# ViTAE-Transformer/SAMRS

Hardware: AMD Instinct MI355X
Metric: images/sec (1024^2, vit_h, 32 boxes/img) SAM box->mask (higher is better)
Workload: dtype f16

## Files before the change

samrs_amd/csrc/engine.hip:

```cpp
#include <algorithm>
#include <cmath>
#include <cstdarg>
#include <cstdio>
#include <cstring>
#include <map>
#include <mutex>
#include <utility>
#include <cstdlib>
#include <string>
#include <vector>

#include "../../include/samrs_hip.h"
#include "../../include/samrs_hip_internal.h"
#include "common.h"
#include "kernels.h"

namespace {

struct DevTensor {
    float* p = nullptr;
    std::vector<int64_t> shape;
    size_t numel = 0;
};

// ... 122 lines not shown

    std::vector<DecLayer> layers;
    DecAttn fin{};
    DecWeights dec{};
    uint16_t* fin_kv_w = nullptr;
    float *fin_kv_b = nullptr, *fin_pe = nullptr;
    uint16_t *up1_w = nullptr, *up2_w = nullptr, *up1_w_lo = nullptr, *up2_w_lo = nullptr;
    float *up1_b = nullptr, *up2_b = nullptr, *up_ln = nullptr;
    float* PE = nullptr;

    float *TOK0 = nullptr, *Q = nullptr, *TA = nullptr, *TQ = nullptr, *TK = nullptr, *TV = nullptr, *TO = nullptr;
    float *MH = nullptr, *QP = nullptr, *KT = nullptr, *VT = nullptr, *O128 = nullptr, *T2IW = nullptr;
    float *K0F = nullptr;
    uint16_t* K0E = nullptr;
    uint16_t* KVQ0 = nullptr;
    float* KF = nullptr;
    uint16_t* KE = nullptr;
    uint16_t* KE_lo = nullptr;
    float* DENSE = nullptr;
    int* SLOT_OF = nullptr;
    uint16_t* KVQ = nullptr;
    uint16_t* OI = nullptr;
    float* U1raw = nullptr;
    uint16_t* U1 = nullptr;
    uint16_t* U2 = nullptr;
    float *HY1 = nullptr, *HY2 = nullptr, *HYPER = nullptr, *IOU = nullptr, *LOW = nullptr;

    void* rle_scratch = nullptr;
    size_t rle_scratch_bytes = 0;
    void* region_scratch = nullptr;
// ... 303 lines not shown
    {
        DeviceGuard dg(device);
        if (dg.status != hipSuccess) return bad("hipSetDevice failed (no HIP device? this library has no CPU fallback)");
    }
    samrs_engine* e = new samrs_engine();
    e->cfg = *cfg;
    e->device = device;
    e->prec = cfg->precision;
    e->grid = cfg->img_size / cfg->patch_size;
    e->tokens = e->grid * e->grid;
    e->D = cfg->embed_dim;
    e->C = cfg->out_chans;
    e->hd = hd;
    e->nwin = (e->grid + cfg->window_size - 1) / cfg->window_size;
    e->T_max = 5 + cfg->max_points + 1 + 2;
    e->slot_set.assign(cfg->max_images, 0);
    e->slot_split.assign(cfg->max_images, 0);
    e->slot_depth.assign(cfg->max_images, 0);
    e->decoder_fusion = env_int("SAMRS_DECODER_FUSION", 1) != 0;
    e->ln_fold = env_int("SAMRS_LN_FOLD", 0) != 0 && gemm_has_experiments();
    const bool h_like = gemm_split3_ok(e->tokens, 3 * e->D, e->D) && gemm_split3_ok(e->tokens, e->D, e->D) && (2 * e->D) % 320 == 0;
    e->split = env_int("SAMRS_SPLIT", SPLIT_DEFAULT | (h_like ? SPLIT_ATTN_V : 0)) & SPLIT_ALL;
    e->grade_multimask = h_like ? SPLIT_ATTN_ANY : 0;
    e->allow_reduced = env_int("SAMRS_ALLOW_REDUCED", getenv("SAMRS_SPLIT") ? 1 : 0) != 0;
    e->upscaler_fused = env_int("SAMRS_UPSCALER_FUSED", 1) != 0;
    e->split_passes = env_int("SAMRS_SPLIT_PASSES", 0) != 0;
    e->split_depth = env_int("SAMRS_SPLIT_DEPTH", 0);
    e->lo_format = (h_like && env_int("SAMRS_LO_FORMAT", 4) == 4) ? 4 : 0;
    e->gelu_fast = env_int("SAMRS_GELU_FAST", -1);
    e->ln_tail = env_int("SAMRS_LN_TAIL", 0) != 0;
// ... 53 lines not shown
        tmp.resize(t.numel);
        for (int64_t ci = 0; ci < Ci; ++ci)
            for (int64_t co = 0; co < Co; ++co)
                for (int64_t s = 0; s < 4; ++s) tmp[(s * Co + co) * Ci + ci] = host[(ci * Co + co) * 4 + s];
        src = tmp.data();
    }
    auto it = e->w.find(n);
    if (it != e->w.end()) return fail(e, SAMRS_ERR_BAD_WEIGHTS, "duplicate tensor %s", name);
    CK(e, dalloc(e, &t.p, t.numel));
    CK(e, hipMemcpy(t.p, src, t.numel * sizeof(float), hipMemcpyHostToDevice));
    e->w.emplace(n, std::move(t));
    return SAMRS_OK;
}

static void audit_build_sites(samrs_engine_t* e);

int samrs_finalize_weights(samrs_engine_t* e, void* stream) {
    if (!e) return SAMRS_ERR_BAD_ARG;
    if (e->finalized) return SAMRS_OK;
    hipStream_t s = (hipStream_t)stream;
    ON_DEVICE(e);
    std::vector<std::pair<std::string, std::vector<int64_t>>> req;
    required_tensors(e, req);
    for (auto& r : req) {
        auto it = e->w.find(r.first);
        if (it == e->w.end()) return fail(e, SAMRS_ERR_BAD_WEIGHTS, "missing tensor %s", r.first.c_str());
        if (it->second.shape != r.second) return fail(e, SAMRS_ERR_BAD_WEIGHTS, "shape mismatch for %s", r.first.c_str());
    }
    if (e->w.size() != req.size()) {
        for (auto& kv : e->w) {
// ... 152 lines not shown
    CK(e, dalloc(e, &e->fin_pe, (size_t)tokens * 2 * Ci));
    CK(e, hipMemsetAsync(e->fin_pe, 0, sizeof(float) * tokens * 2 * Ci, s));
    CK(e, launch_gemm_f32(e->PE, C, e->fin.kw, nullptr, e->fin_pe, 2 * Ci, tokens, Ci, C, false, false, s));
    if ((rc = to_et(e, "mask_decoder.output_upscaling.0.weight", &e->up1_w, false, s, &e->up1_w_lo))) return rc;
    if ((rc = to_et(e, "mask_decoder.output_upscaling.3.weight", &e->up2_w, false, s, &e->up2_w_lo))) return rc;
    CK(e, dalloc(e, &e->up1_b, (size_t)C));
    CK(e, dalloc(e, &e->up2_b, (size_t)C / 2));
    CK(e, dalloc(e, &e->up_ln, (size_t)C / 2));
    CK(e, hipMemcpyAsync(e->up_ln, W(e, "mask_decoder.output_upscaling.1.weight"), sizeof(float) * C / 4, hipMemcpyDeviceToDevice, s));
    CK(e, hipMemcpyAsync(e->up_ln + C / 4, W(e, "mask_decoder.output_upscaling.1.bias"), sizeof(float) * C / 4, hipMemcpyDeviceToDevice, s));
    for (int k = 0; k < 4; ++k) {
        CK(e, hipMemcpyAsync(e->up1_b + k * (C / 4), W(e, "mask_decoder.output_upscaling.0.bias"), sizeof(float) * C / 4, hipMemcpyDeviceToDevice, s));
        CK(e, hipMemcpyAsync(e->up2_b + k * (C / 8), W(e, "mask_decoder.output_upscaling.3.bias"), sizeof(float) * C / 8, hipMemcpyDeviceToDevice, s));
    }

    const size_t Bi = c.max_images, Bb = c.max_prompts;
    const size_t M = Bi * tokens;
    const size_t Mmax = M;
    CK(e, dalloc(e, &e->X, M * D));
    CK(e, dalloc(e, &e->ln_counters, M / 256 + 1));
    CK(e, hipMemsetAsync(e->ln_counters, 0, (M / 256 + 1) * sizeof(unsigned int), s));
    const size_t y_ld_max = e->ldk ? (size_t)e->ldk : (e->outlier_blocks ? (size_t)D + 64 : (size_t)D);
    CK(e, dalloc(e, &e->Y, Mmax * y_ld_max));
    CK(e, hipMemsetAsync(e->Y, 0, Mmax * y_ld_max * 2, s));
    if (e->can_fold) { CK(e, dalloc(e, &e->STATS, Mmax * 16)); CK(e, dalloc(e, &e->ROWSTAT, Mmax * 2)); }
    CK(e, dalloc(e, &e->QKV, Mmax * 3 * D));
    CK(e, dalloc(e, &e->AO, M * D));
    CK(e, dalloc(e, &e->VTG, M * D));
    if (e->oc_resid) {
        CK(e, dalloc(e, &e->OCX, M * 64));
        if (!(e->split & SPLIT_ATTN_ANY)) CK(e, dalloc(e, &e->AOlo, M * D));
// ... 15 lines not shown
                if (!e->Y4[h]) {
                CK(e, dalloc(e, &e->Y4[h], M * D / 2)); CK(e, dalloc(e, &e->SY4[h], mx_scale_bytes((int)M, D, false)));
                }
                CK(e, dalloc(e, &e->AO4[h], M * e->mx_kp_proj / 2)); CK(e, dalloc(e, &e->SAO4[h], mx_scale_bytes((int)M, e->mx_kp_proj, false)));
            }
        }
        if (e->split & SPLIT_MLP) CK(e, dalloc(e, &e->Hlo, M * 4 * D));
    }
    size_t hsz = M * 4 * D;
    if (M * 9 * C * 2 > hsz) hsz = M * 9 * C * 2;
    if (M * 768 > hsz) hsz = M * 768;
    CK(e, dalloc(e, &e->H, hsz));
    CK(e, dalloc(e, &e->N1, M * C));
    CK(e, dalloc(e, &e->N1e, M * C));
    CK(e, dalloc(e, &e->EMB, M * C));
    const size_t BT = Bb * e->T_max;
    CK(e, dalloc(e, &e->TOK0, BT * C)); CK(e, dalloc(e, &e->Q, BT * C)); CK(e, dalloc(e, &e->TA, BT * C));
    CK(e, dalloc(e, &e->TQ, BT * C)); CK(e, dalloc(e, &e->TK, BT * C)); CK(e, dalloc(e, &e->TV, BT * C));
    CK(e, dalloc(e, &e->TO, BT * C)); CK(e, dalloc(e, &e->MH, BT * 2048));
    CK(e, dalloc(e, &e->QP, BT * Ci)); CK(e, dalloc(e, &e->KT, BT * Ci)); CK(e, dalloc(e, &e->VT, BT * Ci));
    CK(e, dalloc(e, &e->O128, BT * Ci));
    CK(e, dalloc(e, &e->T2IW, t2i_workspace_floats(c.max_prompts, e->T_max)));
    CK(e, dalloc(e, &e->K0F, (size_t)c.max_images * tokens * C)); CK(e, dalloc(e, &e->K0E, (size_t)c.max_images * tokens * C));
    CK(e, dalloc(e, &e->KVQ0, (size_t)c.max_images * tokens * 3 * (C / 2)));
    CK(e, dalloc(e, &e->KF, Bb * tokens * C)); CK(e, dalloc(e, &e->KE, Bb * tokens * C));
    CK(e, dalloc(e, &e->KE_lo, Bb * tokens * C));
    CK(e, dalloc(e, &e->KVQ, Bb * tokens * 3 * Ci)); CK(e, dalloc(e, &e->OI, Bb * tokens * Ci));
    CK(e, dalloc(e, &e->U1raw, Bb * tokens * C)); CK(e, dalloc(e, &e->U1, Bb * tokens * C));
    CK(e, dalloc(e, &e->U2, Bb * tokens * 4 * (C / 2)));
    CK(e, dalloc(e, &e->HY1, 5 * Bb * C)); CK(e, dalloc(e, &e->HY2, 5 * Bb * C));
    CK(e, dalloc(e, &e->HYPER, Bb * 4 * (C / 8))); CK(e, dalloc(e, &e->IOU, Bb * 4));
    CK(e, dalloc(e, &e->LOW, Bb * 3 * 256 * 256));
    CK(e, hipStreamSynchronize(s));
    e->dec = dec_weights(e);
    audit_build_sites(e);
    e->finalized = true;
    return SAMRS_OK;
}

static int prepare_slot_keys(samrs_engine_t* e, int slot0, int n, hipStream_t s);

enum { AUDIT_QKV_IN = 0, AUDIT_Q, AUDIT_K, AUDIT_V, AUDIT_PROJ_IN, AUDIT_LIN1_IN, AUDIT_LIN2_IN, AUDIT_PER_BLOCK };
enum { AUDIT_NECK1_IN = 0, AUDIT_NECK2_IN, AUDIT_KEYS0, AUDIT_TAIL };

static void audit_build_sites(samrs_engine_t* e) {
    static const char* const per_block[AUDIT_PER_BLOCK] = {"qkv_in", "q", "k", "v", "proj_in", "lin1_in", "lin2_in"};
    e->audit_sites.clear();
// ... 564 lines not shown
                         : fail(e, SAMRS_ERR_CAPACITY, "slot out of range");
        if (!e->slot_set[slot])
            return multi ? fail(e, SAMRS_ERR_NOT_SET, "An image must be set with .set_image(...) before mask prediction "
                                "(image %d: slot %d is not set).", i, slot)
                         : fail(e, SAMRS_ERR_NOT_SET, "An image must be set with .set_image(...) before mask prediction.");
    }
    if (!boxes && !point_coords && !mask_input) return fail(e, SAMRS_ERR_BAD_ARG, "at least one prompt (points, boxes or mask_input) is required");
    if (point_coords && !point_labels) return fail(e, SAMRS_ERR_BAD_ARG, "point_labels must be supplied if point_coords is supplied.");
    if (point_coords && (n_points < 1 || n_points > c.max_points)) return fail(e, SAMRS_ERR_CAPACITY, "n_points=%d exceeds max_points=%d", n_points, c.max_points);
    for (int i = 0; i < n_img; ++i)
        if (im[i].in_h < 1 || im[i].in_w < 1 || im[i].in_h > c.img_size || im[i].in_w > c.img_size || im[i].orig_h < 1 || im[i].orig_w < 1)
            return multi ? fail(e, SAMRS_ERR_BAD_SHAPE, "image %d: bad input/original size", i) : fail(e, SAMRS_ERR_BAD_SHAPE, "bad input/original size");
    return SAMRS_OK;
}

static int predict_images(samrs_engine_t* e, const PredictImage* im, int n_img, const float* boxes, const float* point_coords,
                          const int32_t* point_labels, int n_points, const float* mask_input, int multimask, int return_logits,
                          float* iou_out, float* lowres_out, void* stream) {
    const int cap = e->cfg.max_prompts;
    const size_t nsel = multimask ? 3 : 1;
    const int np = point_coords ? n_points : 0;
    const int n = n_img ? im[n_img - 1].p1 : 0;
    std::vector<PredictImage> seg;
    int first = 0;
    for (int off = 0; off < n; off += cap) {
        const int m = (n - off) < cap ? (n - off) : cap;
        seg.clear();
        for (int i = first; i < n_img && im[i].p0 < off + m; ++i) {
            const int a = im[i].p0 > off ? im[i].p0 : off, b = im[i].p1 < off + m ? im[i].p1 : off + m;
            if (b <= a) continue;
            PredictImage sgm = im[i];
            const size_t mask_stride = nsel * (size_t)im[i].orig_h * (size_t)im[i].orig_w * (return_logits ? 4 : 1);
            sgm.p0 = a - off; sgm.p1 = b - off;
            sgm.masks = im[i].masks ? (void*)((unsigned char*)im[i].masks + (size_t)(a - im[i].p0) * mask_stride) : nullptr;
// ... 7 lines not shown
            iou_out ? iou_out + (size_t)off * nsel : nullptr, lowres_out ? lowres_out + (size_t)off * nsel * 256 * 256 : nullptr, stream);
        if (rc) return rc;
    }
    return SAMRS_OK;
}

int samrs_predict(samrs_engine_t* e, int slot, int n, const float* boxes, const float* point_coords,
                  const int32_t* point_labels, int n_points, const float* mask_input, int multimask,
                  int return_logits, int in_h, int in_w, int orig_h, int orig_w, void* masks_out, float* iou_out,
                  float* lowres_out, void* stream) {
    if (!e) return SAMRS_ERR_BAD_ARG;
    if (n < 1) return fail(e, SAMRS_ERR_BAD_ARG, "n_prompts must be >= 1");
    if (multimask) { const int rc = check_multimask_grade(e, slot, false); if (rc != SAMRS_OK) return rc; }
    const PredictImage im{slot, 0, n, in_h, in_w, orig_h, orig_w, masks_out};
    { const int rc = check_predict(e, &im, 1, false, boxes, point_coords, point_labels, n_points, mask_input); if (rc != SAMRS_OK) return rc; }
    return predict_images(e, &im, 1, boxes, point_coords, point_labels, n_points, mask_input, multimask, return_logits, iou_out,
                          lowres_out, stream);
}

int samrs_predict_multi(samrs_engine_t* e, int n_images, const int* slots, const int* prompt_offsets, const float* boxes,
                        const float* point_coords, const int32_t* point_labels, int n_points, const float* mask_input, int multimask,
                        int return_logits, const int* in_hw, const int* orig_hw, void* const* masks_out, float* iou_out,
                        float* lowres_out, void* stream) {
    if (!e) return SAMRS_ERR_BAD_ARG;
    if (n_images < 1 || !slots || !prompt_offsets || !in_hw || !orig_hw)
        return fail(e, SAMRS_ERR_BAD_ARG, "samrs_predict_multi: n_images must be >= 1 and slots, prompt_offsets, in_hw, orig_hw non-null");
    if (prompt_offsets[0] != 0) return fail(e, SAMRS_ERR_BAD_ARG, "samrs_predict_multi: prompt_offsets[0] must be 0, got %d", prompt_offsets[0]);
    std::vector<PredictImage> im((size_t)n_images);
    for (int i = 0; i < n_images; ++i) {
        if (prompt_offsets[i + 1] < prompt_offsets[i])
            return fail(e, SAMRS_ERR_BAD_ARG, "samrs_predict_multi: prompt_offsets must not decrease (image %d: %d -> %d)", i,
                        prompt_offsets[i], prompt_offsets[i + 1]);
        im[i] = PredictImage{slots[i], prompt_offsets[i], prompt_offsets[i + 1], in_hw[2 * i], in_hw[2 * i + 1], orig_hw[2 * i],
                             orig_hw[2 * i + 1], masks_out ? masks_out[i] : nullptr};
    }
    if (multimask)
        for (int i = 0; i < n_images; ++i) { const int rc = check_multimask_grade(e, slots[i], true); if (rc != SAMRS_OK) return rc; }
    { const int rc = check_predict(e, im.data(), n_images, true, boxes, point_coords, point_labels, n_points, mask_input); if (rc != SAMRS_OK) return rc; }
    return predict_images(e, im.data(), n_images, boxes, point_coords, point_labels, n_points, mask_input, multimask, return_logits,
                          iou_out, lowres_out, stream);
}

namespace {

enum class I2T { FUSED, PER_SEGMENT, SHARED_RESIDUAL, ACCUMULATE };
enum class Upscaler { ONE_KERNEL, GLN_SPLIT, GLN, UNFUSED };

struct DecodeLayerRoute {
    bool shared = false;
    long bstride = 0;
    bool tab = false;
    I2T i2t = I2T::FUSED;
    bool write_kf = false;
    bool write_ke_lo = false;
// ... 55 lines not shown

static hipError_t ln_tokens(samrs_engine_t* e, int BT, const float* gw, const float* gb, hipStream_t s) {
    return launch_layernorm(e->prec, e->Q, gw, gb, 1e-5f, nullptr, e->Q, BT, e->C, 0, e->grid, 0, s);
}

}

static int run_prompt_side(samrs_engine_t* e, const DecodeRoute& r, const PredictImage* seg, int n_seg, int n, const float* boxes,
                           const float* point_coords, const int32_t* point_labels, int n_points, const float* mask_input, hipStream_t s) {
    const samrs_config& c = e->cfg;
    const int C = e->C, tokens = e->tokens;
    PromptParams pp = e->dec.prompt;
    prompt_call_fields(pp, boxes, point_coords, point_labels, n, n_points, (float)c.img_size);
    CK(e, launch_prompt_tokens(pp, e->TOK0, e->Q, r.T, s));
    if (r.slot_table) {
        if (!e->SLOT_OF) CK(e, dalloc(e, &e->SLOT_OF, (size_t)c.max_prompts));
        std::vector<int> start((size_t)n_seg + 1), slot((size_t)n_seg);
        for (int k = 0; k < n_seg; ++k) { start[k] = seg[k].p0; slot[k] = seg[k].slot; }
        start[n_seg] = seg[n_seg - 1].p1;
        CK(e, launch_fill_slot_table(start.data(), slot.data(), n_seg, e->SLOT_OF, s));
    }
    if (!r.shared0) {
        if (!e->DENSE) CK(e, dalloc(e, &e->DENSE, (size_t)c.max_prompts * tokens * C));
        CK(e, launch_mask_embed(e->dec.mask_embed, mask_input, e->DENSE, n, e->grid, s));
        CK(e, launch_make_keys(e->prec, e->EMB + r.slot0 * tokens * C, e->DENSE, nullptr, e->KF, e->KE, n, tokens, C, s,
                               r.slot_table ? e->SLOT_OF : nullptr));
    }
    return SAMRS_OK;
}

static int run_dec_layer(samrs_engine_t* e, const DecodeRoute& r, int li, const PredictImage* seg, int n_seg, int n, hipStream_t s) {
    const int C = e->C, Ci = C / 2, tokens = e->tokens, prec = e->prec, g = e->grid, T = r.T, BT = r.BT, Mi = r.Mi;
    const DecLayer& L = e->layers[li];
    const DecodeLayerRoute& l = r.layer[li];
    const float* k0f = e->K0F + r.slot0 * tokens * C;
    const uint16_t* kvq = l.shared ? e->KVQ0 + r.slot0 * tokens * 3 * Ci : e->KVQ;
    const int* tab = l.tab ? e->SLOT_OF : nullptr;
    {
// ... 50 lines not shown
}

static int run_final_attn(samrs_engine_t* e, const DecodeRoute& r, int n, hipStream_t s) {
    const int C = e->C, Ci = C / 2, tokens = e->tokens, BT = r.BT;
    CK(e, gemm_f32_sum(e->Q, e->TOK0, C, e->fin.qw, e->fin.qb, e->QP, Ci, BT, Ci, C, s));
    CK(e, launch_gemm_et(e->prec, e->KE, e->fin_kv_w, e->KVQ, e->fin_kv_b, e->fin_pe, tokens, r.Mi, 2 * Ci, C, false, false, false, s));
    CK(e, launch_t2i_attention(e->prec, e->QP, e->KVQ, e->KVQ + Ci, 2 * Ci, tokens, e->O128, e->T2IW, n, r.T, tokens, Ci, 8, s));
    CK(e, launch_gemm_f32(e->O128, Ci, e->fin.ow, e->fin.ob, e->Q, C, BT, C, Ci, false, true, s));
    CK(e, ln_tokens(e, BT, e->dec.norm_final_w, e->dec.norm_final_b, s));
    return SAMRS_OK;
}

static int run_heads(samrs_engine_t* e, const DecodeRoute& r, int n, float* iou_out, hipStream_t s) {
    const int C = e->C;
    const DecWeights& w = e->dec;
    const size_t hs = (size_t)e->cfg.max_prompts * C;
    F32Batch l0{}, l1{}, l2{};
    for (int i = 0; i < 5; ++i) {
        l0.A[i] = i < 4 ? e->Q + (size_t)(1 + i) * C : e->Q;
        l0.W[i] = w.head_w[i][0]; l0.bias[i] = w.head_b[i][0]; l0.C[i] = e->HY1 + i * hs;
        l1.A[i] = e->HY1 + i * hs;
        l1.W[i] = w.head_w[i][1]; l1.bias[i] = w.head_b[i][1]; l1.C[i] = e->HY2 + i * hs;
        if (i < 4) {
            l2.A[i] = e->HY2 + i * hs;
            l2.W[i] = w.head_w[i][2]; l2.bias[i] = w.head_b[i][2]; l2.C[i] = e->HYPER + i * (C / 8);
        }
    }
    CK(e, launch_gemm_f32_batch(l0, 5, r.T * C, C, n, C, C, true, false, s));
    CK(e, launch_gemm_f32_batch(l1, 5, C, C, n, C, C, true, false, s));
    CK(e, launch_gemm_f32_batch(l2, 4, C, 4 * (C / 8), n, C / 8, C, false, false, s));
    if (r.iou)
        CK(e, launch_gemm_f32(e->HY2 + 4 * hs, C, w.head_w[4][2] + (size_t)r.sel0 * C, w.head_b[4][2] + r.sel0, iou_out, r.nsel, n, r.nsel, C,
                              false, false, s));
    return SAMRS_OK;
}

static int run_upscaler(samrs_engine_t* e, const DecodeRoute& r, int n, float* low, hipStream_t s) {
    const int C = e->C, prec = e->prec, g = e->grid, Mi = r.Mi;
    switch (r.up) {
    case Upscaler::ONE_KERNEL:
        CK(e, launch_upscaler_fused(prec, e->KE, r.sp_up ? e->KE_lo : nullptr, e->up1_w, r.sp_up ? e->up1_w_lo : nullptr, e->up1_b, e->up_ln,
                                    e->up2_w, r.sp_up ? e->up2_w_lo : nullptr, e->up2_b, e->HYPER, low, n, g, 4, r.sel0, r.nsel, s));
        break;
    case Upscaler::GLN_SPLIT:
        CK(e, launch_gemm_et_gln(prec, e->KE, e->up1_w, e->U1raw, e->up1_b, e->up_ln, Mi, C, C, s, e->KE_lo, e->up1_w_lo));
        CK(e, launch_upscale2_masks(prec, e->U1raw, e->up2_w, e->up2_w_lo, e->up2_b, e->HYPER, low, n, g, 4, r.sel0, r.nsel, s));
        break;
    case Upscaler::GLN:
        CK(e, launch_gemm_et_gln(prec, e->KE, e->up1_w, e->U1, e->up1_b, e->up_ln, Mi, C, C, s));
        CK(e, launch_upscale2_masks(prec, e->U1, e->up2_w, nullptr, e->up2_b, e->HYPER, low, n, g, 4, r.sel0, r.nsel, s));
        break;
    case Upscaler::UNFUSED:
        CK(e, launch_gemm_et(prec, e->KE, e->up1_w, e->U1raw, e->up1_b, nullptr, 0, Mi, C, C, true, false, false, s));
// ... 5 lines not shown
    return SAMRS_OK;
}

static int run_postprocess(samrs_engine_t* e, const DecodeRoute& r, const PredictImage* seg, int n_seg, const float* low, int return_logits,
                           hipStream_t s) {
    for (int k = 0; k < n_seg; ++k)
        if (seg[k].masks)
            CK(e, launch_postprocess(low + (size_t)seg[k].p0 * r.nsel * 256 * 256, (seg[k].p1 - seg[k].p0) * r.nsel, seg[k].in_h, seg[k].in_w,
                                     seg[k].orig_h, seg[k].orig_w, e->cfg.img_size, return_logits, seg[k].masks, s));
    return SAMRS_OK;
}

static int predict_chunk(samrs_engine_t* e, const PredictImage* seg, int n_seg, int n, const float* boxes, const float* point_coords,
                         const int32_t* point_labels, int n_points, const float* mask_input, int multimask,
                         int return_logits, float* iou_out, float* lowres_out, void* stream) {
    const samrs_config& c = e->cfg;
    if (n < 1 || n > c.max_prompts) return fail(e, SAMRS_ERR_CAPACITY, "n_prompts=%d exceeds max_prompts=%d", n, c.max_prompts);
    hipStream_t s = (hipStream_t)stream;
    ON_DEVICE(e);
    const DecodeRoute r = decode_route(e, n, n_seg, seg[0].slot, boxes != nullptr, point_coords ? n_points : 0, mask_input != nullptr,
                                       multimask != 0, iou_out != nullptr, lowres_out != nullptr);
    float* low = r.low_own ? e->LOW : lowres_out;
    int rc;
    if ((rc = run_prompt_side(e, r, seg, n_seg, n, boxes, point_coords, point_labels, n_points, mask_input, s))) return rc;
    for (int li = 0; li < 2; ++li)
        if ((rc = run_dec_layer(e, r, li, seg, n_seg, n, s))) return rc;
    if ((rc = run_final_attn(e, r, n, s))) return rc;
    if ((rc = run_heads(e, r, n, iou_out, s))) return rc;
    if ((rc = run_upscaler(e, r, n, low, s))) return rc;
    return run_postprocess(e, r, seg, n_seg, low, return_logits, s);
}

// ... 37 lines not shown
    if (!e || !name) return SAMRS_ERR_BAD_ARG;
    const std::string n(name);
    if (n == "decoder_fusion") e->decoder_fusion = value != 0;
    else if (n == "ln_fold") {
        if (value && !gemm_has_experiments())
            return fail(e, SAMRS_ERR_BAD_ARG, "ln_fold: the folded LayerNorm (measured slower: DESIGN.md 6) is built with make EXPERIMENTS=1 only");
        e->ln_fold = value != 0;
    }
    else if (n == "split") {
        if (e->finalized && (value & (SPLIT_ATTN_ANY | SPLIT_MLP | SPLIT_LIN2) & ~e->split_ready))
            return fail(e, SAMRS_ERR_BAD_ARG, "split bits 16 / 32 / 64 / 128 (block GEMMs) need their lo weights: set them before the weights are "
                                              "finalized (SAMRS_SPLIT or options={'split': ...})");
        e->split = value & SPLIT_ALL;
    }
    else if (n == "gemm_variant") e->gemm_variant = value;
    else if (n == "upscaler_fused") e->upscaler_fused = value != 0;
    else if (n == "split_passes") e->split_passes = value != 0;
    else if (n == "split_depth") e->split_depth = value > 0 ? value : 0;
    else if (n == "allow_reduced") e->allow_reduced = value != 0;
    else if (n == "gelu_fast") e->gelu_fast = value < 0 ? -1 : (value != 0);
    else if (n == "ln_tail") e->ln_tail = value > 0;
    else if (n == "operand_pad") e->operand_pad_on = value != 0;
    else if (n == "outlier_cols") e->outlier_on = value & 7;
    else if (n == "outlier_ratio_pct") {
        if (e->finalized) return fail(e, SAMRS_ERR_BAD_ARG, "outlier_ratio_pct: the columns are picked when the weights are finalized; set it before");
        if (value < 101) return fail(e, SAMRS_ERR_BAD_ARG, "outlier_ratio_pct must exceed 100 (a column's score as a percentage of the median score)");
        e->outlier_ratio_pct = value;
    }
    else if (n == "range_check") {
        if (value < 0 || value > 2) return fail(e, SAMRS_ERR_BAD_ARG, "range_check is 0 (off), 1 (count) or 2 (count, and samrs_set_images fails)");
// ... 37 lines not shown
        if (value == 4 && e->finalized && !e->mx_ready && !e->mx_mlp_ready)
            return fail(e, SAMRS_ERR_BAD_ARG, "lo_format 4 needs the fp4 weight copies: set it (and a block-GEMM split bit) before the weights are "
                                              "finalized; it covers the attention-side split of models whose block GEMMs fit the 256 x 320 tile (ViT-H)");
        e->lo_format = value;
    }
    else return fail(e, SAMRS_ERR_BAD_ARG, "unknown option %s", name);
    return SAMRS_OK;
}
int samrs_get_option(const samrs_engine_t* e, const char* name, int* value) {
    if (!e || !name || !value) return SAMRS_ERR_BAD_ARG;
    const std::string n(name);
    if (n == "decoder_fusion") *value = e->decoder_fusion;
    else if (n == "ln_fold") *value = e->ln_fold;
    else if (n == "split") *value = e->split;
    else if (n == "gemm_variant") *value = e->gemm_variant;
    else if (n == "upscaler_fused") *value = e->upscaler_fused;
    else if (n == "split_passes") *value = e->split_passes;
    else if (n == "split_depth") *value = e->split_depth;
    else if (n == "allow_reduced") *value = e->allow_reduced;
    else if (n == "gelu_fast") *value = e->gelu_fast;
    else if (n == "ln_tail") *value = e->ln_tail;
    else if (n == "operand_pad") *value = e->operand_pad_on;
    else if (n == "outlier_cols") *value = e->outlier_on;
    else if (n == "outlier_ratio_pct") *value = e->outlier_ratio_pct;
    else if (n == "outlier_blocks") *value = e->outlier_blocks;
    else if (n == "outlier_columns") *value = e->outlier_columns;
    else if (n == "outlier_dominant_blocks") *value = e->outlier_dominant_blocks;
    else if (n == "range_check") *value = e->range_check;
    else if (n == "saturated") {
        unsigned long long c = 0;
// ... 598 lines not shown
```

samrs_amd/driver.py:

```python
from __future__ import annotations

import contextlib
import os

import queue
import threading
from dataclasses import dataclass, field
from typing import Callable, Iterable, Iterator, List, Optional, Sequence, Tuple

import numpy as np
import torch


def shard(items: Sequence, rank: int, world: int) -> List:
    return list(sorted(items))[rank::world]


def box_chunks(n: int, batch_size: int) -> List[Tuple[int, int]]:
    out, start = [], 0
    end = min(n, start + batch_size)
    for _ in range(n // batch_size + 1):
        if start < end:
            out.append((start, end))
        start = end
# ... 286 lines not shown
        self.png_tab = torch.zeros(batch, 2, 2, dtype=torch.int64).pin_memory() if png else None
        self.png_cur = torch.zeros(1, dtype=torch.int64).pin_memory() if png else None
        self.png_bytes = torch.empty(1 << 20, dtype=torch.uint8).pin_memory() if png else None


QUALITY_OPTIONS = ("quality", "min_stability", "min_pred_iou", "min_inside_box")


def refuse_quality_options(who: str, why: str, **opts) -> None:
    given = [k for k in QUALITY_OPTIONS if opts.get(k)]
    if given:
        raise ValueError(f"{who} does not score masks ({why}): {', '.join(given)} "
                         f"{'is a' if len(given) == 1 else 'are'} TilePipeline option{'' if len(given) == 1 else 's'}")


class TilePipeline:

    BOX_WIDTH = 4

    def __init__(self, sam, n_classes: int, batch: int = 8, box_batch: int = 20, keep_masks: bool = False,
                 out_depth: int = 3, max_boxes: int = 512, device_inputs: bool = False, rle: bool = False,
                 rle_buffer_mb: int = 256, precision="auto", _multimask: bool = False, png_lut: Optional[np.ndarray] = None,
                 png_buffer_mb: Optional[int] = None, batch_decode: bool = False, min_region_area: int = 0,
                 region_mode: str = "both", mask_boxes: bool = False, quality: bool = False, min_stability: float = 0.0,
                 min_pred_iou: float = 0.0, min_inside_box: float = 0.0, polygons: bool = False, polygon_buffer_mb: int = 64,
                 polygon_max_edges: int = 65536):
        from .transforms import ResizeLongestSide
        from .engine import REGION_MODES
        if int(min_region_area) < 0:
            raise ValueError("min_region_area must be >= 0 (0 = off)")
        if region_mode not in REGION_MODES:
            raise ValueError(f"region_mode must be one of {sorted(REGION_MODES)}, got {region_mode!r}")
        self.min_region_area, self.region_mode = int(min_region_area), region_mode
        self.thresholds = (float(min_stability), float(min_pred_iou), float(min_inside_box))
        if any(t != t or t < 0 for t in self.thresholds):
            raise ValueError("min_stability, min_pred_iou and min_inside_box must be >= 0 (0 = off)")
        self.filter = any(t > 0 for t in self.thresholds)
        self.quality = bool(quality) or self.filter
# ... 2 lines not shown
            raise RuntimeError("move the model to the GPU first: sam.to('cuda')")
        self.split_mode = self._choose_split(sam, precision, multimask=_multimask)
        self.allow_reduced = _multimask and isinstance(precision, int) and not isinstance(precision, bool)
        self.eng = eng
        if self.split_mode is not None:
            with self._mode():
                pass
        if out_depth < 2:
            raise ValueError("out_depth must be >= 2: batch k-1's results are still on loan to the sink when batch k decodes")
        if eng.max_images < 2 * batch:
            raise ValueError(f"TilePipeline(batch={batch}) needs an engine with max_images >= {2 * batch} "
                             f"(two embedding slot sets); got {eng.max_images}")
        self.sam, self.eng, self.dev = sam, eng, eng.device
        self.batch, self.box_batch, self.keep_masks, self.max_boxes = batch, box_batch, keep_masks, max_boxes
        self.rle = rle
        self.batch_decode = bool(batch_decode)
        self.png = png_lut is not None
        self.side = sam.cfg.img_size
        self.transform = ResizeLongestSide(sam.image_encoder.img_size)
        self.class_pixels = torch.zeros(n_classes, dtype=torch.int64, device=self.dev)
        self.class_instances = torch.zeros(n_classes, dtype=torch.int64, device=self.dev)
        dev, side = self.dev, self.side
        self.s_h2d, self.s_enc, self.s_dec = (torch.cuda.Stream(dev) for _ in range(3))
        self.device_inputs = device_inputs
        self.pin_in = None
        if not device_inputs:
            self.pin_in = [torch.empty(batch, side, side, 3, dtype=torch.uint8).pin_memory() for _ in range(2)]
        if rle or self.png or polygons:
            self.s_d2h = torch.cuda.Stream(dev)
        if rle:
            self.rle_dev = [torch.empty(rle_buffer_mb << 20, dtype=torch.uint8, device=dev) for _ in range(2)]
# ... 34 lines not shown
            self.poly_cur = [torch.zeros(2, dtype=torch.int64, device=dev) for _ in range(2)]
            self.poly_tab = [torch.zeros(batch * max_boxes, 5, dtype=torch.int64, device=dev) for _ in range(2)]
        if self.quality:
            self.cnt_dev = [torch.zeros(batch, max_boxes, 4, dtype=torch.int64, device=dev) for _ in range(2)]
            self.keep_dev = [torch.ones(batch, max_boxes, dtype=torch.uint8, device=dev) for _ in range(2)]
            self.qual_dev = [torch.zeros(batch, max_boxes, dtype=torch.float32, device=dev) for _ in range(2)]
        self.ev_h2d = [torch.cuda.Event() for _ in range(2)]
        self.ev_enc = [torch.cuda.Event() for _ in range(2)]
        self.ev_dec = [torch.cuda.Event() for _ in range(2)]
        self.ev_in_free = [torch.cuda.Event() for _ in range(2)]
        self.free_out: "queue.Queue[_OutBuf]" = queue.Queue()
        for _ in range(out_depth):
            self.free_out.put(_OutBuf(batch, side, max_boxes, rle, self.png, self.min_region_area > 0, self.mask_boxes, self.quality,
                                      self.polygons))

    @staticmethod
    def _choose_split(sam, precision, multimask: bool) -> Optional[int]:
        from .engine import SPLIT_DEFAULT
        if precision == "engine":
            return None
        if precision == "auto":
            if "split" in getattr(sam, "options", {}) or "SAMRS_SPLIT" in os.environ:
                return None
            return int(getattr(sam, "default_split", SPLIT_DEFAULT)) if multimask else SPLIT_DEFAULT
        return int(precision)

    @contextlib.contextmanager
    def _mode(self):
        if self.split_mode is None:
            yield
# ... 506 lines not shown
```

samrs_amd/generate.py:

```python
from __future__ import annotations

import argparse
import json
import os
import pickle
from typing import Dict, List, Optional, Sequence, Tuple

import numpy as np
import torch

from . import driver, quality, rle, tile_io


def default_palette(n_classes: int) -> np.ndarray:
    rng = np.random.default_rng(12345)
    return rng.integers(0, 256, size=(n_classes, 3), dtype=np.uint8)


class StageClock:

    def __init__(self) -> None:
        self.t: Dict[str, float] = {}
        self.n: Dict[str, int] = {}

# ... 219 lines not shown
    poly_kw = dict(polygons=True, polygon_buffer_mb=int(getattr(args, "polygon_buffer_mb", 64) or 64),
                   polygon_max_edges=int(getattr(args, "polygon_max_edges", 65536) or 65536)) if want_polygons else {}
    if scene_window > 0:
        from . import scene
        pipe = scene.ScenePipeline(sam, n_classes, window=scene_window, overlap=getattr(args, "scene_overlap", 256),
                                   context=getattr(args, "scene_context", 2.0), batch=batch, box_batch=args.box_batch,
                                   rle=not args.no_rle, rle_buffer_mb=getattr(args, "rle_buffer_mb", 256),
                                   png_lut=tile_io.class_lut(palette) if png_device else None,
                                   min_region_area=min_region_area, region_mode=getattr(args, "region_mode", "both"),
                                   mask_boxes=mask_boxes, quality=want_quality, **thresholds, **poly_kw)
    else:
        pipe = driver.TilePipeline(sam, n_classes, batch=batch, box_batch=args.box_batch, rle=not args.no_rle,
                                   rle_buffer_mb=getattr(args, "rle_buffer_mb", 256), max_boxes=max_boxes,
                                   out_depth=getattr(args, "out_depth", 4), png_lut=tile_io.class_lut(palette) if png_device else None,
                                   png_buffer_mb=getattr(args, "png_buffer_mb", None),
                                   batch_decode=bool(getattr(args, "batch_decode", False)),
                                   min_region_area=min_region_area, region_mode=getattr(args, "region_mode", "both"),
                                   mask_boxes=mask_boxes, quality=want_quality, **thresholds, **poly_kw)
    import zlib
    wq_name = "samrs_wq/%08x/%d" % (zlib.crc32("\n".join(stems).encode()), _RUN_SEQ[0])
    _RUN_SEQ[0] += 1
    wq = driver.WorkQueue(len(stems), chunk=batch, rank=rank, world=world, mode=getattr(args, "schedule", "static"), name=wq_name)

    import time
    tile_io.load_library()
    n_readers, n_writers = io_threads(getattr(args, "readers", 0) or 0, getattr(args, "writers", 0) or 0, png_device=png_device)
    warn = host_bound_warning(n_readers, n_writers, png_device=png_device)
    if warn:
        import sys
        print(f"[rank {rank}] warning: {warn}", file=sys.stderr, flush=True)
    png_level = getattr(args, "png_level", tile_io.LEVEL_LABELS)
# ... 290 lines not shown
```

samrs_amd/instances.py:

```python
from __future__ import annotations

import argparse
import json
import math
import os
import xml.etree.ElementTree as ET
from dataclasses import dataclass
from typing import Dict, List, Optional, Sequence, Tuple

import numpy as np

TAGS = {"point": "hbox", "rbox_mask": "rbox", "box": "rhbox"}
IMAGE_EXTS = (".png", ".jpg", ".jpeg", ".tif", ".bmp")


@dataclass
class HrscImage:
    hboxes: np.ndarray
    rboxes: np.ndarray
    colors: np.ndarray
    points: np.ndarray
    skip: bool


# ... 180 lines not shown
    if getattr(args, "resume", False):
        todo = driver.agree_on_list(pending_stems(args.out, stems) if rank == 0 else [])
        if rank == 0:
            print(f"[rank 0] --resume: {len(stems) - len(todo)} of {len(stems)} images already complete", flush=True)
    batch = getattr(args, "batch", 8)
    multimask = bool(getattr(args, "multimask", False))
    split = getattr(args, "split", None)
    opts = generate.default_split_options(split) if not multimask else ({"split": int(split)} if split is not None else None)
    sam = samrs_amd.sam_model_registry[args.model](checkpoint=args.checkpoint, precision=getattr(args, "precision", "f16"), options=opts,
                                                   audit_passes=getattr(args, "audit_passes", 0),
                                                   max_images=2 * batch, max_prompts=args.box_batch).to(f"cuda:{local}")
    max_boxes = max([len(anns[s].colors) for s in stems] + [1])
    pipe = driver.InstancePipeline(sam, 1, prompt=args.prompt, multimask=multimask, fill_rule=getattr(args, "fill_rule", "auto"),
                                   gt=with_gt, batch=batch, box_batch=args.box_batch, max_boxes=max_boxes, rle=True,
                                   rle_buffer_mb=getattr(args, "rle_buffer_mb", 256), keep_masks=False,
                                   batch_decode=bool(getattr(args, "batch_decode", False)),
                                   min_region_area=int(getattr(args, "min_region_area", 0) or 0),
                                   region_mode=getattr(args, "region_mode", "both"),
                                   mask_boxes=bool(getattr(args, "mask_boxes", False)))
    os.makedirs(os.path.join(args.out, "parts"), exist_ok=True)
    import zlib
    wq_name = "samrs_ins/%08x" % zlib.crc32(("\n".join(todo) + "|" + args.out).encode())
    wq = driver.WorkQueue(len(todo), chunk=batch, rank=rank, world=world, mode=getattr(args, "schedule", "static"), name=wq_name)

    def load(stem: str) -> driver.WorkItem:
        a = anns[stem]
        img = tile_io.read_rgb(os.path.join(args.images, files[stem]))
        ann = a.points if args.prompt == "point" else a.rboxes
        gt = None
        if with_gt:
            gt = (tile_io.read_rgb(os.path.join(args.gt_labels, stem + ".png")), a.colors)
# ... 88 lines not shown
```

Measured before the change: 145.4.

## Auto-enable batched decode and grow decoder workspaces to fit whole batch

Decoder workspaces are now sized by a runtime decode_prompts option instead of max_prompts, and can be reallocated larger on request (up to 512 prompts). The tile pipeline now turns batch_decode on by default ('auto') when every image fits in one chunk, raising decode_prompts so a whole batch's boxes go through one decoder chain. The aim is fewer, larger decoder launches in place of per-image ones. In exchange it uses more device memory and adds a device sync when workspaces are reallocated.

```diff
diff --git a/samrs_amd/csrc/engine.hip b/samrs_amd/csrc/engine.hip
--- a/samrs_amd/csrc/engine.hip
+++ b/samrs_amd/csrc/engine.hip
@@ -160,6 +160,9 @@
     float *K0F = nullptr;
     uint16_t* K0E = nullptr;
     uint16_t* KVQ0 = nullptr;
+    int decode_prompts = 0;
+    int decode_alloc = 0;
+    size_t decode_bytes = 0;
     float* KF = nullptr;
     uint16_t* KE = nullptr;
     uint16_t* KE_lo = nullptr;
@@ -493,6 +496,7 @@
     e->hd = hd;
     e->nwin = (e->grid + cfg->window_size - 1) / cfg->window_size;
     e->T_max = 5 + cfg->max_points + 1 + 2;
+    e->decode_prompts = cfg->max_prompts;
     e->slot_set.assign(cfg->max_images, 0);
     e->slot_split.assign(cfg->max_images, 0);
     e->slot_depth.assign(cfg->max_images, 0);
@@ -576,6 +580,81 @@
 }
 
 static void audit_build_sites(samrs_engine_t* e);
+
+constexpr int DECODE_PROMPTS_LIMIT = 512;
+
+struct DecodeBuf {
+    const char* name;
+    size_t per_prompt;
+    bool lazy;
+    void* (*get)(const samrs_engine_t*);
+    void (*set)(samrs_engine_t*, void*);
+};
+#define DECODE_BUF(field, elems, lazy)                                                             \
+    DecodeBuf{#field, sizeof(*static_cast<samrs_engine_t*>(nullptr)->field) * (size_t)(elems), lazy, \
+              [](const samrs_engine_t* e) -> void* { return e->field; },                           \
+              [](samrs_engine_t* e, void* p) { e->field = static_cast<decltype(e->field)>(p); }}
+
+static std::vector<DecodeBuf> decode_buffers(const samrs_engine_t* e) {
+    const size_t T = (size_t)e->T_max, tokens = (size_t)e->tokens, C = (size_t)e->C, Ci = C / 2;
+    return {
+        DECODE_BUF(TOK0, T * C, false), DECODE_BUF(Q, T * C, false), DECODE_BUF(TA, T * C, false), DECODE_BUF(TQ, T * C, false),
+        DECODE_BUF(TK, T * C, false), DECODE_BUF(TV, T * C, false), DECODE_BUF(TO, T * C, false), DECODE_BUF(MH, T * 2048, false),
+        DECODE_BUF(QP, T * Ci, false), DECODE_BUF(KT, T * Ci, false), DECODE_BUF(VT, T * Ci, false), DECODE_BUF(O128, T * Ci, false),
+        DECODE_BUF(T2IW, t2i_workspace_floats(1, e->T_max), false),
+        DECODE_BUF(KF, tokens * C, false), DECODE_BUF(KE, tokens * C, false), DECODE_BUF(KE_lo, tokens * C, false),
+        DECODE_BUF(KVQ, tokens * 3 * Ci, false), DECODE_BUF(OI, tokens * Ci, false),
+        DECODE_BUF(DENSE, tokens * C, true), DECODE_BUF(SLOT_OF, 1, true),
+        DECODE_BUF(U1raw, tokens * C, true), DECODE_BUF(U1, tokens * C, true), DECODE_BUF(U2, tokens * 4 * Ci, true),
+        DECODE_BUF(HY1, 5 * C, false), DECODE_BUF(HY2, 5 * C, false), DECODE_BUF(HYPER, 4 * (C / 8), false), DECODE_BUF(IOU, 4, false),
+        DECODE_BUF(LOW, 3 * 256 * 256, false),
+    };
+}
+#undef DECODE_BUF
+
+static int grow_decode_workspaces(samrs_engine_t* e, int cap) {
+    if (cap <= e->decode_alloc) return SAMRS_OK;
+    const std::vector<DecodeBuf> bufs = decode_buffers(e);
+    std::vector<void*> fresh(bufs.size(), nullptr);
+    size_t bytes = 0;
+    for (size_t i = 0; i < bufs.size(); ++i) {
+        if (bufs[i].lazy && !bufs[i].get(e)) continue;
+        const hipError_t r = hipMalloc(&fresh[i], bufs[i].per_prompt * (size_t)cap);
+        if (r != hipSuccess) {
+            for (void* p : fresh) if (p) (void)hipFree(p);
+            return fail(e, SAMRS_ERR_HIP, "decoder workspaces for %d prompts: %s (%zu bytes for %s)", cap, hipGetErrorString(r),
+                        bufs[i].per_prompt * (size_t)cap, bufs[i].name);
+        }
+        bytes += bufs[i].per_prompt * (size_t)cap;
+    }
+    if (e->decode_alloc > 0) CK(e, hipDeviceSynchronize());
+    for (size_t i = 0; i < bufs.size(); ++i) {
+        if (!fresh[i]) continue;
+        if (void* old = bufs[i].get(e)) {
+            e->owned.erase(std::find(e->owned.begin(), e->owned.end(), old));
+            (void)hipFree(old);
+        }
+        e->owned.push_back(fresh[i]);
+        bufs[i].set(e, fresh[i]);
+    }
+    e->decode_alloc = cap;
+    e->decode_bytes = bytes;
+    return SAMRS_OK;
+}
+
+static int need_decode_buffer(samrs_engine_t* e, const char* name) {
+    for (const DecodeBuf& b : decode_buffers(e)) {
+        if (strcmp(b.name, name)) continue;
+        if (b.get(e)) return SAMRS_OK;
+        void* p = nullptr;
+        CK(e, hipMalloc(&p, b.per_prompt * (size_t)e->decode_alloc));
+        e->owned.push_back(p);
+        b.set(e, p);
+        e->decode_bytes += b.per_prompt * (size_t)e->decode_alloc;
+        return SAMRS_OK;
+    }
+    return fail(e, SAMRS_ERR_BAD_ARG, "no decoder workspace named %s", name);
+}
 
 int samrs_finalize_weights(samrs_engine_t* e, void* stream) {
     if (!e) return SAMRS_ERR_BAD_ARG;
@@ -758,7 +837,7 @@
         CK(e, hipMemcpyAsync(e->up2_b + k * (C / 8), W(e, "mask_decoder.output_upscaling.3.bias"), sizeof(float) * C / 8, hipMemcpyDeviceToDevice, s));
     }
 
-    const size_t Bi = c.max_images, Bb = c.max_prompts;
+    const size_t Bi = c.max_images;
     const size_t M = Bi * tokens;
     const size_t Mmax = M;
     CK(e, dalloc(e, &e->X, M * D));
@@ -804,23 +883,9 @@
     CK(e, dalloc(e, &e->N1, M * C));
     CK(e, dalloc(e, &e->N1e, M * C));
     CK(e, dalloc(e, &e->EMB, M * C));
-    const size_t BT = Bb * e->T_max;
-    CK(e, dalloc(e, &e->TOK0, BT * C)); CK(e, dalloc(e, &e->Q, BT * C)); CK(e, dalloc(e, &e->TA, BT * C));
-    CK(e, dalloc(e, &e->TQ, BT * C)); CK(e, dalloc(e, &e->TK, BT * C)); CK(e, dalloc(e, &e->TV, BT * C));
-    CK(e, dalloc(e, &e->TO, BT * C)); CK(e, dalloc(e, &e->MH, BT * 2048));
-    CK(e, dalloc(e, &e->QP, BT * Ci)); CK(e, dalloc(e, &e->KT, BT * Ci)); CK(e, dalloc(e, &e->VT, BT * Ci));
-    CK(e, dalloc(e, &e->O128, BT * Ci));
-    CK(e, dalloc(e, &e->T2IW, t2i_workspace_floats(c.max_prompts, e->T_max)));
     CK(e, dalloc(e, &e->K0F, (size_t)c.max_images * tokens * C)); CK(e, dalloc(e, &e->K0E, (size_t)c.max_images * tokens * C));
     CK(e, dalloc(e, &e->KVQ0, (size_t)c.max_images * tokens * 3 * (C / 2)));
-    CK(e, dalloc(e, &e->KF, Bb * tokens * C)); CK(e, dalloc(e, &e->KE, Bb * tokens * C));
-    CK(e, dalloc(e, &e->KE_lo, Bb * tokens * C));
-    CK(e, dalloc(e, &e->KVQ, Bb * tokens * 3 * Ci)); CK(e, dalloc(e, &e->OI, Bb * tokens * Ci));
-    CK(e, dalloc(e, &e->U1raw, Bb * tokens * C)); CK(e, dalloc(e, &e->U1, Bb * tokens * C));
-    CK(e, dalloc(e, &e->U2, Bb * tokens * 4 * (C / 2)));
-    CK(e, dalloc(e, &e->HY1, 5 * Bb * C)); CK(e, dalloc(e, &e->HY2, 5 * Bb * C));
-    CK(e, dalloc(e, &e->HYPER, Bb * 4 * (C / 8))); CK(e, dalloc(e, &e->IOU, Bb * 4));
-    CK(e, dalloc(e, &e->LOW, Bb * 3 * 256 * 256));
+    if ((rc = grow_decode_workspaces(e, e->decode_prompts))) return rc;
     CK(e, hipStreamSynchronize(s));
     e->dec = dec_weights(e);
     audit_build_sites(e);
@@ -1415,10 +1480,9 @@
     return SAMRS_OK;
 }
 
-static int predict_images(samrs_engine_t* e, const PredictImage* im, int n_img, const float* boxes, const float* point_coords,
+static int predict_images(samrs_engine_t* e, int cap, const PredictImage* im, int n_img, const float* boxes, const float* point_coords,
                           const int32_t* point_labels, int n_points, const float* mask_input, int multimask, int return_logits,
                           float* iou_out, float* lowres_out, void* stream) {
-    const int cap = e->cfg.max_prompts;
     const size_t nsel = multimask ? 3 : 1;
     const int np = point_coords ? n_points : 0;
     const int n = n_img ? im[n_img - 1].p1 : 0;
@@ -1456,7 +1520,7 @@
     if (multimask) { const int rc = check_multimask_grade(e, slot, false); if (rc != SAMRS_OK) return rc; }
     const PredictImage im{slot, 0, n, in_h, in_w, orig_h, orig_w, masks_out};
     { const int rc = check_predict(e, &im, 1, false, boxes, point_coords, point_labels, n_points, mask_input); if (rc != SAMRS_OK) return rc; }
-    return predict_images(e, &im, 1, boxes, point_coords, point_labels, n_points, mask_input, multimask, return_logits, iou_out,
+    return predict_images(e, e->cfg.max_prompts, &im, 1, boxes, point_coords, point_labels, n_points, mask_input, multimask, return_logits, iou_out,
                           lowres_out, stream);
 }
 
@@ -1479,7 +1543,7 @@
     if (multimask)
         for (int i = 0; i < n_images; ++i) { const int rc = check_multimask_grade(e, slots[i], true); if (rc != SAMRS_OK) return rc; }
     { const int rc = check_predict(e, im.data(), n_images, true, boxes, point_coords, point_labels, n_points, mask_input); if (rc != SAMRS_OK) return rc; }
-    return predict_images(e, im.data(), n_images, boxes, point_coords, point_labels, n_points, mask_input, multimask, return_logits,
+    return predict_images(e, e->decode_prompts, im.data(), n_images, boxes, point_coords, point_labels, n_points, mask_input, multimask, return_logits,
                           iou_out, lowres_out, stream);
 }
 
@@ -1565,14 +1629,14 @@
     prompt_call_fields(pp, boxes, point_coords, point_labels, n, n_points, (float)c.img_size);
     CK(e, launch_prompt_tokens(pp, e->TOK0, e->Q, r.T, s));
     if (r.slot_table) {
-        if (!e->SLOT_OF) CK(e, dalloc(e, &e->SLOT_OF, (size_t)c.max_prompts));
+        if (!e->SLOT_OF) { const int rc = need_decode_buffer(e, "SLOT_OF"); if (rc != SAMRS_OK) return rc; }
         std::vector<int> start((size_t)n_seg + 1), slot((size_t)n_seg);
         for (int k = 0; k < n_seg; ++k) { start[k] = seg[k].p0; slot[k] = seg[k].slot; }
         start[n_seg] = seg[n_seg - 1].p1;
         CK(e, launch_fill_slot_table(start.data(), slot.data(), n_seg, e->SLOT_OF, s));
     }
     if (!r.shared0) {
-        if (!e->DENSE) CK(e, dalloc(e, &e->DENSE, (size_t)c.max_prompts * tokens * C));
+        if (!e->DENSE) { const int rc = need_decode_buffer(e, "DENSE"); if (rc != SAMRS_OK) return rc; }
         CK(e, launch_mask_embed(e->dec.mask_embed, mask_input, e->DENSE, n, e->grid, s));
         CK(e, launch_make_keys(e->prec, e->EMB + r.slot0 * tokens * C, e->DENSE, nullptr, e->KF, e->KE, n, tokens, C, s,
                                r.slot_table ? e->SLOT_OF : nullptr));
@@ -1653,7 +1717,7 @@
 static int run_heads(samrs_engine_t* e, const DecodeRoute& r, int n, float* iou_out, hipStream_t s) {
     const int C = e->C;
     const DecWeights& w = e->dec;
-    const size_t hs = (size_t)e->cfg.max_prompts * C;
+    const size_t hs = (size_t)e->decode_alloc * C;
     F32Batch l0{}, l1{}, l2{};
     for (int i = 0; i < 5; ++i) {
         l0.A[i] = i < 4 ? e->Q + (size_t)(1 + i) * C : e->Q;
@@ -1676,6 +1740,11 @@
 
 static int run_upscaler(samrs_engine_t* e, const DecodeRoute& r, int n, float* low, hipStream_t s) {
     const int C = e->C, prec = e->prec, g = e->grid, Mi = r.Mi;
+    for (const char* name : {"U1raw", "U1", "U2"}) {
+        const bool used = !strcmp(name, "U1raw") ? (r.up == Upscaler::GLN_SPLIT || r.up == Upscaler::UNFUSED)
+                        : !strcmp(name, "U1")    ? (r.up == Upscaler::GLN || r.up == Upscaler::UNFUSED) : r.up == Upscaler::UNFUSED;
+        if (used) { const int rc = need_decode_buffer(e, name); if (rc != SAMRS_OK) return rc; }
+    }
     switch (r.up) {
     case Upscaler::ONE_KERNEL:
         CK(e, launch_upscaler_fused(prec, e->KE, r.sp_up ? e->KE_lo : nullptr, e->up1_w, r.sp_up ? e->up1_w_lo : nullptr, e->up1_b, e->up_ln,
@@ -1711,8 +1780,8 @@
 static int predict_chunk(samrs_engine_t* e, const PredictImage* seg, int n_seg, int n, const float* boxes, const float* point_coords,
                          const int32_t* point_labels, int n_points, const float* mask_input, int multimask,
                          int return_logits, float* iou_out, float* lowres_out, void* stream) {
-    const samrs_config& c = e->cfg;
-    if (n < 1 || n > c.max_prompts) return fail(e, SAMRS_ERR_CAPACITY, "n_prompts=%d exceeds max_prompts=%d", n, c.max_prompts);
+    if (n < 1 || n > e->decode_prompts || n > e->decode_alloc)
+        return fail(e, SAMRS_ERR_CAPACITY, "a decoder chain of %d prompts exceeds decode_prompts=%d", n, e->decode_prompts);
     hipStream_t s = (hipStream_t)stream;
     ON_DEVICE(e);
     const DecodeRoute r = decode_route(e, n, n_seg, seg[0].slot, boxes != nullptr, point_coords ? n_points : 0, mask_input != nullptr,
@@ -1780,6 +1849,19 @@
         e->split = value & SPLIT_ALL;
     }
     else if (n == "gemm_variant") e->gemm_variant = value;
+    else if (n == "decode_prompts") {
+        const long long prod = (long long)e->cfg.max_images * e->cfg.max_prompts;
+        const int lo = e->cfg.max_prompts, lim = prod < DECODE_PROMPTS_LIMIT ? (int)prod : DECODE_PROMPTS_LIMIT, hi = lim > lo ? lim : lo;
+        if (value < lo || value > hi)
+            return fail(e, SAMRS_ERR_BAD_ARG, "decode_prompts=%d is outside [%d, %d]: from max_prompts to max_images x max_prompts = %lld, "
+                                              "at most %d (the index range of the decoder kernels)", value, lo, hi, prod, DECODE_PROMPTS_LIMIT);
+        if (e->finalized) {
+            ON_DEVICE(e);
+            const int rc = grow_decode_workspaces(e, value);
+            if (rc != SAMRS_OK) return rc;
+        }
+        e->decode_prompts = value;
+    }
     else if (n == "upscaler_fused") e->upscaler_fused = value != 0;
     else if (n == "split_passes") e->split_passes = value != 0;
     else if (n == "split_depth") e->split_depth = value > 0 ? value : 0;
@@ -1847,6 +1929,8 @@
     else if (n == "ln_fold") *value = e->ln_fold;
     else if (n == "split") *value = e->split;
     else if (n == "gemm_variant") *value = e->gemm_variant;
+    else if (n == "decode_prompts") *value = e->decode_prompts;
+    else if (n == "decode_kbytes") *value = (int)((e->decode_bytes + 1023) / 1024);
     else if (n == "upscaler_fused") *value = e->upscaler_fused;
     else if (n == "split_passes") *value = e->split_passes;
     else if (n == "split_depth") *value = e->split_depth;
diff --git a/samrs_amd/driver.py b/samrs_amd/driver.py
--- a/samrs_amd/driver.py
+++ b/samrs_amd/driver.py
@@ -324,6 +324,24 @@
                          f"{'is a' if len(given) == 1 else 'are'} TilePipeline option{'' if len(given) == 1 else 's'}")
 
 
+DECODE_PROMPTS_LIMIT = 512
+
+
+def resolve_batch_decode(batch_decode, batch: int, box_batch: int, max_boxes: int, max_prompts: int, max_images: int,
+                         capacity: int) -> Tuple[bool, Optional[int], str]:
+    if batch_decode != "auto":
+        return bool(batch_decode), None, "explicit"
+    if box_batch < max_boxes:
+        return False, None, f"box_batch={box_batch} < max_boxes={max_boxes}: tiles are decoded in several chunks"
+    need = batch * max_boxes
+    if need <= capacity:
+        return True, None, f"a chain of {need} prompts fits the engine's decode_prompts={capacity}"
+    hi = min(max_images * max_prompts, DECODE_PROMPTS_LIMIT)
+    if need > hi:
+        return False, None, f"a chain of {need} prompts exceeds what the engine accepts ({hi})"
+    return True, need, f"decode_prompts raised from {capacity} to {need}"
+
+
 class TilePipeline:
 
     BOX_WIDTH = 4
@@ -331,7 +349,7 @@
     def __init__(self, sam, n_classes: int, batch: int = 8, box_batch: int = 20, keep_masks: bool = False,
                  out_depth: int = 3, max_boxes: int = 512, device_inputs: bool = False, rle: bool = False,
                  rle_buffer_mb: int = 256, precision="auto", _multimask: bool = False, png_lut: Optional[np.ndarray] = None,
-                 png_buffer_mb: Optional[int] = None, batch_decode: bool = False, min_region_area: int = 0,
+                 png_buffer_mb: Optional[int] = None, batch_decode="auto", min_region_area: int = 0,
                  region_mode: str = "both", mask_boxes: bool = False, quality: bool = False, min_stability: float = 0.0,
                  min_pred_iou: float = 0.0, min_inside_box: float = 0.0, polygons: bool = False, polygon_buffer_mb: int = 64,
                  polygon_max_edges: int = 65536):
@@ -364,7 +382,8 @@
         self.sam, self.eng, self.dev = sam, eng, eng.device
         self.batch, self.box_batch, self.keep_masks, self.max_boxes = batch, box_batch, keep_masks, max_boxes
         self.rle = rle
-        self.batch_decode = bool(batch_decode)
+        self.batch_decode, self.batch_decode_reason = self._resolve_batch_decode(batch_decode)
+        self.batch_decode_on = self.batch_decode
         self.png = png_lut is not None
         self.side = sam.cfg.img_size
         self.transform = ResizeLongestSide(sam.image_encoder.img_size)
@@ -429,6 +448,23 @@
             self.free_out.put(_OutBuf(batch, side, max_boxes, rle, self.png, self.min_region_area > 0, self.mask_boxes, self.quality,
                                       self.polygons))
 
+    def _resolve_batch_decode(self, batch_decode) -> Tuple[bool, str]:
+        from .engine import EngineError
+        if batch_decode != "auto":
+            return bool(batch_decode), "explicit"
+        eng = self.eng
+        try:
+            capacity = eng.get_option("decode_prompts")
+        except (AssertionError, EngineError):
+            capacity = eng.max_prompts
+        on, want, why = resolve_batch_decode("auto", self.batch, self.box_batch, self.max_boxes, eng.max_prompts, eng.max_images, capacity)
+        if on and want is not None:
+            try:
+                eng.set_option("decode_prompts", want)
+            except (AssertionError, EngineError) as exc:
+                return False, f"the engine refused decode_prompts={want}: {exc}"
+        return on, why
+
     @staticmethod
     def _choose_split(sam, precision, multimask: bool) -> Optional[int]:
         from .engine import SPLIT_DEFAULT
diff --git a/samrs_amd/generate.py b/samrs_amd/generate.py
--- a/samrs_amd/generate.py
+++ b/samrs_amd/generate.py
@@ -257,7 +257,7 @@
                                    rle_buffer_mb=getattr(args, "rle_buffer_mb", 256), max_boxes=max_boxes,
                                    out_depth=getattr(args, "out_depth", 4), png_lut=tile_io.class_lut(palette) if png_device else None,
                                    png_buffer_mb=getattr(args, "png_buffer_mb", None),
-                                   batch_decode=bool(getattr(args, "batch_decode", False)),
+                                   batch_decode=True if getattr(args, "batch_decode", False) else "auto",
                                    min_region_area=min_region_area, region_mode=getattr(args, "region_mode", "both"),
                                    mask_boxes=mask_boxes, quality=want_quality, **thresholds, **poly_kw)
     import zlib
diff --git a/samrs_amd/instances.py b/samrs_amd/instances.py
--- a/samrs_amd/instances.py
+++ b/samrs_amd/instances.py
@@ -218,7 +218,7 @@
     pipe = driver.InstancePipeline(sam, 1, prompt=args.prompt, multimask=multimask, fill_rule=getattr(args, "fill_rule", "auto"),
                                    gt=with_gt, batch=batch, box_batch=args.box_batch, max_boxes=max_boxes, rle=True,
                                    rle_buffer_mb=getattr(args, "rle_buffer_mb", 256), keep_masks=False,
-                                   batch_decode=bool(getattr(args, "batch_decode", False)),
+                                   batch_decode=True if getattr(args, "batch_decode", False) else "auto",
                                    min_region_area=int(getattr(args, "min_region_area", 0) or 0),
                                    region_mode=getattr(args, "region_mode", "both"),
                                    mask_boxes=bool(getattr(args, "mask_boxes", False)))
```

Measured after the change: 147.3 (median of 6 runs). 1.01x the previous value.
